# EternityJune25/ComoRAG

Hardware: NVIDIA H100
Metric: queries/sec (higher is better)
Workload: dtype bf16

## Files before the change

comorag_b200/csrc/common.cu:

```cuda
#include "common.cuh"

#include <stdarg.h>
#include <string.h>

#include <mutex>

namespace crag {

namespace {
thread_local char g_err[512] = {0};

typedef CUresult (*EncodeTiledFn)(CUtensorMap*, CUtensorMapDataType, cuuint32_t, void*, const cuuint64_t*,
                                  const cuuint64_t*, const cuuint32_t*, const cuuint32_t*, CUtensorMapInterleave,
                                  CUtensorMapSwizzle, CUtensorMapL2promotion, CUtensorMapFloatOOBfill);

EncodeTiledFn get_encode_fn() {
  static EncodeTiledFn fn = nullptr;
  static std::once_flag once;
  std::call_once(once, [] {
    void* p = nullptr;
    cudaDriverEntryPointQueryResult q;
    if (cudaGetDriverEntryPoint("cuTensorMapEncodeTiled", &p, cudaEnableDefault, &q) == cudaSuccess &&
        q == cudaDriverEntryPointSuccess)
      fn = reinterpret_cast<EncodeTiledFn>(p);
  });
  return fn;
}
}

void set_error(const char* fmt, ...) {
  va_list ap;
  va_start(ap, fmt);
  vsnprintf(g_err, sizeof(g_err), fmt, ap);
  va_end(ap);
}

int fail(int code, const char* fmt, ...) {
  va_list ap;
  va_start(ap, fmt);
  vsnprintf(g_err, sizeof(g_err), fmt, ap);
  va_end(ap);
  return code;
}

int make_tmap_bf16_2d(CUtensorMap* out, const void* base, uint64_t rows, uint64_t cols, uint64_t row_stride_bytes,
                      uint32_t box_rows, uint32_t box_cols) {
  EncodeTiledFn enc = get_encode_fn();
  if (!enc) return fail(CRAG_ERR_CUDA, "cuTensorMapEncodeTiled entry point unavailable (driver too old?)");
  if (rows == 0 || cols == 0) return fail(CRAG_ERR_INVALID, "tensor map over an empty tensor");
  const cuuint64_t gdim[2] = {cols, rows};
  const cuuint64_t gstride[1] = {row_stride_bytes};
  const cuuint32_t box[2] = {box_cols, box_rows};
  const cuuint32_t estride[2] = {1, 1};
  CUresult r = enc(out, CU_TENSOR_MAP_DATA_TYPE_BFLOAT16, 2, const_cast<void*>(base), gdim, gstride, box, estride,
                   CU_TENSOR_MAP_INTERLEAVE_NONE, CU_TENSOR_MAP_SWIZZLE_128B, CU_TENSOR_MAP_L2_PROMOTION_L2_256B,
                   CU_TENSOR_MAP_FLOAT_OOB_FILL_NONE);
  if (r != CUDA_SUCCESS)
    return fail(CRAG_ERR_CUDA, "cuTensorMapEncodeTiled failed (CUresult %d; rows=%llu cols=%llu stride=%llu box=%ux%u)",
                int(r), (unsigned long long)rows, (unsigned long long)cols, (unsigned long long)row_stride_bytes,
                box_rows, box_cols);
  return CRAG_OK;
}

int sm_count() {
  static int cached[64] = {0};
  int dev = 0;
  cudaError_t e = cudaGetDevice(&dev);
  if (e != cudaSuccess || dev < 0 || dev >= 64) {
    fail(CRAG_ERR_CUDA, "no usable CUDA device (%s)", e != cudaSuccess ? cudaGetErrorString(e) : "device ordinal out of range");
    return -1;
  }
  if (cached[dev] == 0) {
    int n = 0;
    e = cudaDeviceGetAttribute(&n, cudaDevAttrMultiProcessorCount, dev);
    if (e != cudaSuccess) {
      fail(CRAG_ERR_CUDA, "cudaDeviceGetAttribute: %s", cudaGetErrorString(e));
      return -1;
    }
    cached[dev] = n;
  }
  return cached[dev];
}

}

extern "C" int crag_version(void) { return 1002; }
extern "C" const char* crag_last_error(void) { return crag::g_err; }
extern "C" int crag_sm_count(void) { return crag::sm_count(); }

namespace crag {
namespace {
struct VmemApi {
  CUresult (*reserve)(CUdeviceptr*, size_t, size_t, CUdeviceptr, unsigned long long) = nullptr;
  CUresult (*addr_free)(CUdeviceptr, size_t) = nullptr;
  CUresult (*create)(CUmemGenericAllocationHandle*, size_t, const CUmemAllocationProp*, unsigned long long) = nullptr;
  CUresult (*release)(CUmemGenericAllocationHandle) = nullptr;
  CUresult (*map)(CUdeviceptr, size_t, size_t, CUmemGenericAllocationHandle, unsigned long long) = nullptr;
  CUresult (*unmap)(CUdeviceptr, size_t) = nullptr;
  CUresult (*set_access)(CUdeviceptr, size_t, const CUmemAccessDesc*, size_t) = nullptr;
  CUresult (*granularity)(size_t*, const CUmemAllocationProp*, CUmemAllocationGranularity_flags) = nullptr;
  bool ok = false;
};

const VmemApi& vmem_api() {
  static VmemApi api;
  static std::once_flag once;
  std::call_once(once, [] {
    auto get = [](const char* name, void** fn) {
      cudaDriverEntryPointQueryResult q;
      return cudaGetDriverEntryPoint(name, fn, cudaEnableDefault, &q) == cudaSuccess && q == cudaDriverEntryPointSuccess;
    };
    api.ok = get("cuMemAddressReserve", reinterpret_cast<void**>(&api.reserve)) &&
             get("cuMemAddressFree", reinterpret_cast<void**>(&api.addr_free)) &&
             get("cuMemCreate", reinterpret_cast<void**>(&api.create)) &&
             get("cuMemRelease", reinterpret_cast<void**>(&api.release)) &&
             get("cuMemMap", reinterpret_cast<void**>(&api.map)) &&
             get("cuMemUnmap", reinterpret_cast<void**>(&api.unmap)) &&
             get("cuMemSetAccess", reinterpret_cast<void**>(&api.set_access)) &&
             get("cuMemGetAllocationGranularity", reinterpret_cast<void**>(&api.granularity));
  });
  return api;
}

CUmemAllocationProp vmem_prop(int dev) {
  CUmemAllocationProp prop = {};
  prop.type = CU_MEM_ALLOCATION_TYPE_PINNED;
  prop.location.type = CU_MEM_LOCATION_TYPE_DEVICE;
  prop.location.id = dev;
  return prop;
}
}
}

extern "C" int crag_vmem_reserve(size_t max_bytes, uint64_t* base_out, size_t* granularity_out) {
  using namespace crag;
  const VmemApi& api = vmem_api();
  if (!api.ok) return fail(CRAG_ERR_UNSUPPORTED, "virtual memory management entry points unavailable");
  if (!base_out || !granularity_out || max_bytes == 0) return fail(CRAG_ERR_INVALID, "crag_vmem_reserve: bad arguments");
  int dev = 0;
  CRAG_CUDA_OK(cudaGetDevice(&dev));
  CRAG_CUDA_OK(cudaFree(nullptr));
  const CUmemAllocationProp prop = vmem_prop(dev);
  size_t gran = 0;
  CUresult r = api.granularity(&gran, &prop, CU_MEM_ALLOC_GRANULARITY_RECOMMENDED);
  if (r != CUDA_SUCCESS || gran == 0) return fail(CRAG_ERR_CUDA, "cuMemGetAllocationGranularity failed (%d)", int(r));
  const size_t size = (max_bytes + gran - 1) / gran * gran;
  CUdeviceptr base = 0;
  r = api.reserve(&base, size, gran, 0, 0);
  if (r != CUDA_SUCCESS) return fail(CRAG_ERR_CUDA, "cuMemAddressReserve(%zu) failed (%d)", size, int(r));
  *base_out = uint64_t(base);
  *granularity_out = gran;
  return CRAG_OK;
}

extern "C" int crag_vmem_grow(uint64_t base, size_t mapped_bytes, size_t new_mapped_bytes) {
  using namespace crag;
  const VmemApi& api = vmem_api();
  if (!api.ok) return fail(CRAG_ERR_UNSUPPORTED, "virtual memory management entry points unavailable");
  if (new_mapped_bytes <= mapped_bytes) return CRAG_OK;
  int dev = 0;
  CRAG_CUDA_OK(cudaGetDevice(&dev));
  const CUmemAllocationProp prop = vmem_prop(dev);
  const size_t bytes = new_mapped_bytes - mapped_bytes;
  CUmemGenericAllocationHandle h;
  CUresult r = api.create(&h, bytes, &prop, 0);
  if (r != CUDA_SUCCESS) return fail(CRAG_ERR_CUDA, "cuMemCreate(%zu) failed (%d): out of device memory?", bytes, int(r));
  r = api.map(CUdeviceptr(base + mapped_bytes), bytes, 0, h, 0);
  if (r != CUDA_SUCCESS) {
    api.release(h);
    return fail(CRAG_ERR_CUDA, "cuMemMap failed (%d)", int(r));
  }
  api.release(h);
  CUmemAccessDesc acc = {};
  acc.location.type = CU_MEM_LOCATION_TYPE_DEVICE;
  acc.location.id = dev;
  acc.flags = CU_MEM_ACCESS_FLAGS_PROT_READWRITE;
  r = api.set_access(CUdeviceptr(base + mapped_bytes), bytes, &acc, 1);
  if (r != CUDA_SUCCESS) return fail(CRAG_ERR_CUDA, "cuMemSetAccess failed (%d)", int(r));
  return CRAG_OK;
}

extern "C" int crag_vmem_release(uint64_t base, size_t mapped_bytes, size_t reserved_bytes) {
  using namespace crag;
  const VmemApi& api = vmem_api();
  if (!api.ok) return fail(CRAG_ERR_UNSUPPORTED, "virtual memory management entry points unavailable");
  if (mapped_bytes) {
    CUresult r = api.unmap(CUdeviceptr(base), mapped_bytes);
    if (r != CUDA_SUCCESS) return fail(CRAG_ERR_CUDA, "cuMemUnmap failed (%d)", int(r));
  }
  CUresult r = api.addr_free(CUdeviceptr(base), reserved_bytes);
  if (r != CUDA_SUCCESS) return fail(CRAG_ERR_CUDA, "cuMemAddressFree failed (%d)", int(r));
  return CRAG_OK;
}
```

comorag_b200/csrc/gemm.cu:

```cuda
#include <cstdlib>

#include "common.cuh"
#include "gemm.cuh"
#include "ptx.cuh"

namespace crag {

constexpr int kGemmBM = 128;
constexpr int kGemmBN = 128;
constexpr int kGemmBK = 64;
constexpr int kGemmConsumerWarps = 8;
constexpr int kGemmThreads = 32 * kGemmConsumerWarps + 32;
constexpr int kGemmStages = 3;

struct GemmLayout {
  static constexpr int kABytes = kGemmBM * kGemmBK * 2;
  static constexpr int kBBytes = kGemmBN * kGemmBK * 2;
  static constexpr int kStageBytes = kABytes + kBBytes;
  static constexpr size_t smem_bytes() { return 1024 + size_t(kGemmStages) * kStageBytes + 2 * kGemmStages * 8; }
};

__device__ __forceinline__ float gelu_erf(float x) {
  const float z = x * 0.70710678118654752f;
  const float az = fabsf(z);
  float t;
  asm("rcp.approx.ftz.f32 %0, %1;" : "=f"(t) : "f"(fmaf(0.3275911f, az, 1.0f)));
  float p = fmaf(1.061405429f, t, -1.453152027f);
  p = fmaf(p, t, 1.421413741f);
  p = fmaf(p, t, -0.284496736f);
  p = fmaf(p, t, 0.254829592f);
  p *= t;
  float e;
  asm("ex2.approx.ftz.f32 %0, %1;" : "=f"(e) : "f"(az * az * -1.4426950408889634f));
  const float erf_abs = fmaf(-p, e, 1.0f);
  const float half_x = 0.5f * x;
  return fmaf(half_x, copysignf(erf_abs, z), half_x);
}

__device__ __forceinline__ uint32_t pack_bf16x2(float a, float b) {
  __nv_bfloat162 v = __floats2bfloat162_rn(a, b);
  return *reinterpret_cast<uint32_t*>(&v);
}

template <int EPI>
__global__ void __launch_bounds__(kGemmThreads, 2)
gemm_bf16_kernel(const __grid_constant__ CUtensorMap tm_a, const __grid_constant__ CUtensorMap tm_b, int M, int N,
                 int K, const float* __restrict__ bias, const __nv_bfloat16* __restrict__ residual, int64_t ldr,
                 __nv_bfloat16* __restrict__ out, int64_t ldo) {
  using L = GemmLayout;
  constexpr int STAGES = kGemmStages;
  extern __shared__ uint8_t smem_raw[];
  uint8_t* smem = reinterpret_cast<uint8_t*>((reinterpret_cast<uintptr_t>(smem_raw) + 1023) & ~uintptr_t(1023));
  uint64_t* bar_full = reinterpret_cast<uint64_t*>(smem + STAGES * L::kStageBytes);
  uint64_t* bar_empty = bar_full + STAGES;

  const int warp = threadIdx.x >> 5;
  const int lane = threadIdx.x & 31;
  int n_blk = blockIdx.x, m_blk = blockIdx.y;
  if constexpr (EPI == GEMM_EPI_SCORES_F32) {
    const int m_blocks = (M + kGemmBM - 1) / kGemmBM;
    m_blk = int(blockIdx.x % unsigned(m_blocks));
    n_blk = int(blockIdx.x / unsigned(m_blocks));
  }
  const int num_kb = (K + kGemmBK - 1) / kGemmBK;

  if (threadIdx.x == 0) {
    for (int s = 0; s < STAGES; ++s) {
      mbar_init(&bar_full[s], 1);
      mbar_init(&bar_empty[s], kGemmConsumerWarps);
    }
    fence_mbar_init();
  }
  __syncthreads();

  if (warp == kGemmConsumerWarps) {
    if (lane == 0) {
      tma_prefetch_desc(&tm_a);
      tma_prefetch_desc(&tm_b);
      const uint64_t pol_w = policy_evict_last();
      int stage = 0;
      uint32_t phase = 0;
      for (int kb = 0; kb < num_kb; ++kb) {
        mbar_wait(&bar_empty[stage], phase ^ 1);
        uint8_t* sa = smem + stage * L::kStageBytes;
        mbar_arrive_expect_tx(&bar_full[stage], L::kStageBytes);
        tma_load_2d(&tm_a, &bar_full[stage], sa, kb * kGemmBK, m_blk * kGemmBM);
        tma_load_2d_hint(&tm_b, &bar_full[stage], sa + L::kABytes, kb * kGemmBK, n_blk * kGemmBN, pol_w);
        if (++stage == STAGES) { stage = 0; phase ^= 1; }
      }
    }
    return;
  }

  const int wg = warp >> 2;
  float acc[kGemmBN / 2];
#pragma unroll
  for (int i = 0; i < kGemmBN / 2; ++i) acc[i] = 0.f;
  int stage = 0, prev = 0;
  uint32_t phase = 0;
  for (int kb = 0; kb < num_kb; ++kb) {
    mbar_wait(&bar_full[stage], phase);
    const uint32_t a_addr = smem_u32(smem + stage * L::kStageBytes) + wg * 64 * 128;
    const uint32_t b_addr = smem_u32(smem + stage * L::kStageBytes + L::kABytes);
    wgmma_fence();
#pragma unroll
    for (int ks = 0; ks < kGemmBK / 16; ++ks)
      wgmma_m64n128k16_ss(acc, wgmma_desc_sw128(a_addr + ks * 32), wgmma_desc_sw128(b_addr + ks * 32), 1u);
    wgmma_commit();
    wgmma_wait<1>();
    if (kb > 0 && lane == 0) mbar_arrive(&bar_empty[prev]);
    prev = stage;
    if (++stage == STAGES) { stage = 0; phase ^= 1; }
  }
  wgmma_wait<0>();
  wgmma_fence_regs(acc);

  if constexpr (EPI == GEMM_EPI_SCORES_F32) {
    float* outf = reinterpret_cast<float*>(out);
    const int srow0 = m_blk * kGemmBM + wg * 64 + (warp & 3) * 16 + (lane >> 2);
    const int scol0 = n_blk * kGemmBN + 2 * (lane & 3);
#pragma unroll
    for (int j = 0; j < kGemmBN / 8; ++j) {
      const int col = scol0 + 8 * j;
#pragma unroll
      for (int h = 0; h < 2; ++h) {
        const int row = srow0 + 8 * h;
        if (row >= M) continue;
        float* p = outf + int64_t(row) * ldo + col;
        if (col + 1 < N) *reinterpret_cast<float2*>(p) = make_float2(acc[4 * j + 2 * h], acc[4 * j + 2 * h + 1]);
        else if (col < N) p[0] = acc[4 * j + 2 * h];
      }
    }
    return;
  }

  const int row0 = m_blk * kGemmBM + wg * 64 + (warp & 3) * 16 + (lane >> 2);
  const int col0 = n_blk * kGemmBN + 2 * (lane & 3);
#pragma unroll
  for (int j = 0; j < kGemmBN / 8; ++j) {
    const int col = col0 + 8 * j;
    if (col >= N) continue;
    const float2 b = __ldg(reinterpret_cast<const float2*>(bias + col));
#pragma unroll
    for (int h = 0; h < 2; ++h) {
      const int row = row0 + 8 * h;
      if (row >= M) continue;
      float x0 = acc[4 * j + 2 * h] + b.x, x1 = acc[4 * j + 2 * h + 1] + b.y;
      if (EPI == GEMM_EPI_BIAS_GELU) {
        x0 = gelu_erf(x0);
        x1 = gelu_erf(x1);
      }
      if (EPI == GEMM_EPI_BIAS_RESIDUAL) {
        const __nv_bfloat162 r = *reinterpret_cast<const __nv_bfloat162*>(residual + int64_t(row) * ldr + col);
        x0 += __bfloat162float(r.x);
        x1 += __bfloat162float(r.y);
      }
      *reinterpret_cast<uint32_t*>(out + int64_t(row) * ldo + col) = pack_bf16x2(x0, x1);
    }
  }
}

template <int EPI>
static int launch_gemm_t(const CUtensorMap& tm_a, const CUtensorMap& tm_b, int M, int N, int K, const float* bias,
                         const __nv_bfloat16* residual, int64_t ldr, __nv_bfloat16* out, int64_t ldo,
                         cudaStream_t stream) {
  auto kern = gemm_bf16_kernel<EPI>;
  {
    static bool done[64] = {false};
    int dev = 0;
    CRAG_CUDA_OK(cudaGetDevice(&dev));
    if (dev < 0 || dev >= 64 || !done[dev]) {
      CRAG_CUDA_OK(cudaFuncSetAttribute(kern, cudaFuncAttributeMaxDynamicSharedMemorySize, int(GemmLayout::smem_bytes())));
      if (dev >= 0 && dev < 64) done[dev] = true;
    }
  }
  const unsigned n_blocks = (N + kGemmBN - 1) / kGemmBN, m_blocks = (M + kGemmBM - 1) / kGemmBM;
  const dim3 grid = EPI == GEMM_EPI_SCORES_F32 ? dim3(m_blocks * n_blocks) : dim3(n_blocks, m_blocks);
  kern<<<grid, kGemmThreads, GemmLayout::smem_bytes(), stream>>>(tm_a, tm_b, M, N, K, bias, residual, ldr, out, ldo);
  CRAG_CUDA_OK(cudaGetLastError());
  return CRAG_OK;
}

int gemm_bf16(const void* a, int64_t lda, const void* w, int64_t ldw, const float* bias, const void* residual,
              int64_t ldr, void* out, int64_t ldo, int M, int N, int K, int epi, cudaStream_t stream) {
  if (M <= 0) return CRAG_OK;
  if (N < 8 || K < 8 || N % 8 != 0 || K % 8 != 0) return fail(CRAG_ERR_INVALID, "gemm: N and K must be positive multiples of 8 (N=%d K=%d)", N, K);
  if (lda % 8 || ldw % 8 || ldo % 8 || (epi == GEMM_EPI_BIAS_RESIDUAL && ldr % 8)) return fail(CRAG_ERR_INVALID, "gemm: leading dimensions must be multiples of 8 elements");
  if (!a || !w || !bias || !out || (epi == GEMM_EPI_BIAS_RESIDUAL && !residual)) return fail(CRAG_ERR_INVALID, "gemm: null pointer");
  if ((uintptr_t(a) | uintptr_t(w) | uintptr_t(out) | uintptr_t(bias) | uintptr_t(residual)) & 15) return fail(CRAG_ERR_INVALID, "gemm: pointers must be 16-byte aligned");
  if ((M + kGemmBM - 1) / kGemmBM > 65535) return fail(CRAG_ERR_INVALID, "gemm: M too large (%d)", M);
  const __nv_bfloat16* res = static_cast<const __nv_bfloat16*>(residual);
  __nv_bfloat16* o = static_cast<__nv_bfloat16*>(out);
  CUtensorMap tm_a, tm_b;
  int rc = make_tmap_bf16_2d(&tm_a, a, uint64_t(M), uint64_t(K), uint64_t(lda) * 2, kGemmBM);
  if (rc != CRAG_OK) return rc;
  rc = make_tmap_bf16_2d(&tm_b, w, uint64_t(N), uint64_t(K), uint64_t(ldw) * 2, kGemmBN);
  if (rc != CRAG_OK) return rc;
  switch (epi) {
    case GEMM_EPI_BIAS: return launch_gemm_t<GEMM_EPI_BIAS>(tm_a, tm_b, M, N, K, bias, res, ldr, o, ldo, stream);
    case GEMM_EPI_BIAS_GELU: return launch_gemm_t<GEMM_EPI_BIAS_GELU>(tm_a, tm_b, M, N, K, bias, res, ldr, o, ldo, stream);
    case GEMM_EPI_BIAS_RESIDUAL: return launch_gemm_t<GEMM_EPI_BIAS_RESIDUAL>(tm_a, tm_b, M, N, K, bias, res, ldr, o, ldo, stream);
  }
  return fail(CRAG_ERR_INVALID, "gemm: unknown epilogue %d", epi);
}

int gemm_scores_f32(const void* a, int64_t lda, const void* w, int64_t ldw, float* out, int64_t ldo, int M, int N,
                    int K, cudaStream_t stream) {
  if (M <= 0 || N <= 0) return CRAG_OK;
  if (K < 64 || K % 64 != 0 || lda % 8 || ldw % 8 || ldo % 2) return fail(CRAG_ERR_INVALID, "gemm scores: K must be a multiple of 64, lda/ldw multiples of 8 and ldo even");
  if ((uintptr_t(a) | uintptr_t(w)) & 15 || uintptr_t(out) & 7) return fail(CRAG_ERR_INVALID, "gemm scores: misaligned pointer");
  if (int64_t((M + kGemmBM - 1) / kGemmBM) * ((N + kGemmBN - 1) / kGemmBN) > int64_t(0x7FFFFFFF)) return fail(CRAG_ERR_INVALID, "gemm scores: too many tiles (M=%d N=%d)", M, N);
  CUtensorMap tm_a, tm_b;
  int rc = make_tmap_bf16_2d(&tm_a, a, uint64_t(M), uint64_t(K), uint64_t(lda) * 2, kGemmBM);
  if (rc != CRAG_OK) return rc;
  rc = make_tmap_bf16_2d(&tm_b, w, uint64_t(N), uint64_t(K), uint64_t(ldw) * 2, kGemmBN);
  if (rc != CRAG_OK) return rc;
  return launch_gemm_t<GEMM_EPI_SCORES_F32>(tm_a, tm_b, M, N, K, nullptr, nullptr, 0, reinterpret_cast<__nv_bfloat16*>(out),
                                            ldo, stream);
}

}

extern "C" int crag_gemm_bf16(const void* a, int64_t lda, const void* w, int64_t ldw, const float* bias,
                              const void* residual, int64_t ldr, void* out, int64_t ldo, int m, int n, int k,
                              int epilogue, crag_stream_t stream) {
  return crag::gemm_bf16(a, lda, w, ldw, bias, residual, ldr, out, ldo, m, n, k, epilogue,
                         static_cast<cudaStream_t>(stream));
}
```

comorag_b200/csrc/ptx.cuh:

```cuda
#pragma once
#include <cuda.h>
#include <cuda_runtime.h>
#include <cuda_bf16.h>
#include <stdint.h>

namespace crag {

__device__ __forceinline__ uint32_t smem_u32(const void* p) {
  return static_cast<uint32_t>(__cvta_generic_to_shared(p));
}

__device__ __forceinline__ bool elect_one() {
  uint32_t pred = 0;
  asm volatile(
      "{\n\t.reg .pred p;\n\t"
      "elect.sync _|p, 0xffffffff;\n\t"
      "selp.u32 %0, 1, 0, p;\n\t}"
      : "=r"(pred));
  return pred != 0;
}

__device__ __forceinline__ void mbar_init(uint64_t* bar, uint32_t count) {
  asm volatile("mbarrier.init.shared::cta.b64 [%0], %1;" ::"r"(smem_u32(bar)), "r"(count));
}
__device__ __forceinline__ void fence_mbar_init() {
  asm volatile("fence.mbarrier_init.release.cluster;" ::: "memory");
}
__device__ __forceinline__ void fence_proxy_async() {
  asm volatile("fence.proxy.async.shared::cta;" ::: "memory");
}
__device__ __forceinline__ void mbar_arrive_expect_tx(uint64_t* bar, uint32_t bytes) {
  asm volatile("mbarrier.arrive.expect_tx.shared::cta.b64 _, [%0], %1;" ::"r"(smem_u32(bar)), "r"(bytes)
               : "memory");
}
__device__ __forceinline__ void mbar_arrive(uint64_t* bar) {
  asm volatile("mbarrier.arrive.shared::cta.b64 _, [%0];" ::"r"(smem_u32(bar)) : "memory");
}
__device__ __forceinline__ bool mbar_try_wait(uint64_t* bar, uint32_t parity) {
  uint32_t ok;
  asm volatile(
      "{\n\t.reg .pred p;\n\t"
      "mbarrier.try_wait.parity.shared::cta.b64 p, [%1], %2;\n\t"
      "selp.u32 %0, 1, 0, p;\n\t}"
      : "=r"(ok)
      : "r"(smem_u32(bar)), "r"(parity)
      : "memory");
  return ok != 0;
}
#ifndef CRAG_MBAR_SPIN_LIMIT
#define CRAG_MBAR_SPIN_LIMIT (1ll << 33)
#endif
__device__ __forceinline__ void mbar_wait(uint64_t* bar, uint32_t parity) {
  if (mbar_try_wait(bar, parity)) return;
  const long long t0 = clock64();
  uint32_t spins = 0;
  while (!mbar_try_wait(bar, parity)) {
    if ((++spins & 0x3FF) == 0 && clock64() - t0 > CRAG_MBAR_SPIN_LIMIT) __trap();
  }
}

__device__ __forceinline__ void tma_prefetch_desc(const CUtensorMap* m) {
  asm volatile("prefetch.tensormap [%0];" ::"l"(reinterpret_cast<uint64_t>(m)) : "memory");
}
__device__ __forceinline__ void tma_load_2d(const CUtensorMap* m, uint64_t* bar, void* dst, int32_t c0,
                                            int32_t c1) {
  asm volatile(
      "cp.async.bulk.tensor.2d.shared::cluster.global.mbarrier::complete_tx::bytes"
      " [%0], [%1, {%3, %4}], [%2];" ::"r"(smem_u32(dst)),
      "l"(reinterpret_cast<uint64_t>(m)), "r"(smem_u32(bar)), "r"(c0), "r"(c1)
      : "memory");
}
__device__ __forceinline__ void tma_load_2d_hint(const CUtensorMap* m, uint64_t* bar, void* dst, int32_t c0,
                                                 int32_t c1, uint64_t policy) {
  asm volatile(
      "cp.async.bulk.tensor.2d.shared::cluster.global.mbarrier::complete_tx::bytes.L2::cache_hint"
      " [%0], [%1, {%3, %4}], [%2], %5;" ::"r"(smem_u32(dst)),
      "l"(reinterpret_cast<uint64_t>(m)), "r"(smem_u32(bar)), "r"(c0), "r"(c1), "l"(policy)
      : "memory");
}
__device__ __forceinline__ uint64_t policy_evict_first() {
  uint64_t p;
  asm volatile("createpolicy.fractional.L2::evict_first.b64 %0, 1.0;" : "=l"(p));
  return p;
}
__device__ __forceinline__ uint64_t policy_evict_normal() {
  uint64_t p;
  asm volatile("createpolicy.fractional.L2::evict_normal.b64 %0, 1.0;" : "=l"(p));
  return p;
}
__device__ __forceinline__ uint64_t policy_evict_last() {
  uint64_t p;
  asm volatile("createpolicy.fractional.L2::evict_last.b64 %0, 1.0;" : "=l"(p));
  return p;
}

__device__ __forceinline__ void wgmma_fence() { asm volatile("wgmma.fence.sync.aligned;" ::: "memory"); }
__device__ __forceinline__ void wgmma_commit() { asm volatile("wgmma.commit_group.sync.aligned;" ::: "memory"); }
template <int N>
__device__ __forceinline__ void wgmma_wait() { asm volatile("wgmma.wait_group.sync.aligned %0;" ::"n"(N) : "memory"); }
template <int R>
__device__ __forceinline__ void wgmma_fence_regs(float (&d)[R]) {
#pragma unroll
  for (int i = 0; i < R; ++i) asm volatile("" : "+f"(d[i])::"memory");
}

__device__ __forceinline__ uint64_t wgmma_desc_sw128(uint32_t smem_addr) {
  uint64_t d = 0;
  d |= static_cast<uint64_t>((smem_addr & 0x3FFFF) >> 4);
  d |= static_cast<uint64_t>(1) << 16;
  d |= static_cast<uint64_t>(1024 >> 4) << 32;
  d |= static_cast<uint64_t>(1) << 62;
  return d;
}

__device__ __forceinline__ void wgmma_m64n32k16_ss(float (&d)[16], uint64_t desc_a, uint64_t desc_b, uint32_t accumulate) {
  asm volatile(
      "{\n\t.reg .pred p;\n\t"
      "setp.ne.b32 p, %18, 0;\n\t"
      "wgmma.mma_async.sync.aligned.m64n32k16.f32.bf16.bf16 "
      "{%0, %1, %2, %3, %4, %5, %6, %7, %8, %9, %10, %11, %12, %13, %14, %15}, %16, %17, p, 1, 1, 0, 0;\n\t}"
      : "+f"(d[0]), "+f"(d[1]), "+f"(d[2]), "+f"(d[3]), "+f"(d[4]), "+f"(d[5]), "+f"(d[6]), "+f"(d[7]), "+f"(d[8]), "+f"(d[9]), "+f"(d[10]), "+f"(d[11]), "+f"(d[12]), "+f"(d[13]), "+f"(d[14]), "+f"(d[15])
      : "l"(desc_a), "l"(desc_b), "r"(accumulate));
}
__device__ __forceinline__ void wgmma_m64n64k16_ss(float (&d)[32], uint64_t desc_a, uint64_t desc_b, uint32_t accumulate) {
  asm volatile(
      "{\n\t.reg .pred p;\n\t"
      "setp.ne.b32 p, %34, 0;\n\t"
      "wgmma.mma_async.sync.aligned.m64n64k16.f32.bf16.bf16 "
      "{%0, %1, %2, %3, %4, %5, %6, %7, %8, %9, %10, %11, %12, %13, %14, %15, %16, %17, %18, %19, %20, %21, %22, %23, %24, %25, %26, %27, %28, %29, %30, %31}, %32, %33, p, 1, 1, 0, 0;\n\t}"
      : "+f"(d[0]), "+f"(d[1]), "+f"(d[2]), "+f"(d[3]), "+f"(d[4]), "+f"(d[5]), "+f"(d[6]), "+f"(d[7]), "+f"(d[8]), "+f"(d[9]), "+f"(d[10]), "+f"(d[11]), "+f"(d[12]), "+f"(d[13]), "+f"(d[14]), "+f"(d[15]), "+f"(d[16]), "+f"(d[17]), "+f"(d[18]), "+f"(d[19]), "+f"(d[20]), "+f"(d[21]), "+f"(d[22]), "+f"(d[23]), "+f"(d[24]), "+f"(d[25]), "+f"(d[26]), "+f"(d[27]), "+f"(d[28]), "+f"(d[29]), "+f"(d[30]), "+f"(d[31])
      : "l"(desc_a), "l"(desc_b), "r"(accumulate));
}
__device__ __forceinline__ void wgmma_m64n128k16_ss(float (&d)[64], uint64_t desc_a, uint64_t desc_b, uint32_t accumulate) {
  asm volatile(
      "{\n\t.reg .pred p;\n\t"
      "setp.ne.b32 p, %66, 0;\n\t"
      "wgmma.mma_async.sync.aligned.m64n128k16.f32.bf16.bf16 "
      "{%0, %1, %2, %3, %4, %5, %6, %7, %8, %9, %10, %11, %12, %13, %14, %15, %16, %17, %18, %19, %20, %21, %22, %23, %24, %25, %26, %27, %28, %29, %30, %31, %32, %33, %34, %35, %36, %37, %38, %39, %40, %41, %42, %43, %44, %45, %46, %47, %48, %49, %50, %51, %52, %53, %54, %55, %56, %57, %58, %59, %60, %61, %62, %63}, %64, %65, p, 1, 1, 0, 0;\n\t}"
      : "+f"(d[0]), "+f"(d[1]), "+f"(d[2]), "+f"(d[3]), "+f"(d[4]), "+f"(d[5]), "+f"(d[6]), "+f"(d[7]), "+f"(d[8]), "+f"(d[9]), "+f"(d[10]), "+f"(d[11]), "+f"(d[12]), "+f"(d[13]), "+f"(d[14]), "+f"(d[15]), "+f"(d[16]), "+f"(d[17]), "+f"(d[18]), "+f"(d[19]), "+f"(d[20]), "+f"(d[21]), "+f"(d[22]), "+f"(d[23]), "+f"(d[24]), "+f"(d[25]), "+f"(d[26]), "+f"(d[27]), "+f"(d[28]), "+f"(d[29]), "+f"(d[30]), "+f"(d[31]), "+f"(d[32]), "+f"(d[33]), "+f"(d[34]), "+f"(d[35]), "+f"(d[36]), "+f"(d[37]), "+f"(d[38]), "+f"(d[39]), "+f"(d[40]), "+f"(d[41]), "+f"(d[42]), "+f"(d[43]), "+f"(d[44]), "+f"(d[45]), "+f"(d[46]), "+f"(d[47]), "+f"(d[48]), "+f"(d[49]), "+f"(d[50]), "+f"(d[51]), "+f"(d[52]), "+f"(d[53]), "+f"(d[54]), "+f"(d[55]), "+f"(d[56]), "+f"(d[57]), "+f"(d[58]), "+f"(d[59]), "+f"(d[60]), "+f"(d[61]), "+f"(d[62]), "+f"(d[63])
      : "l"(desc_a), "l"(desc_b), "r"(accumulate));
}
__device__ __forceinline__ void wgmma_m64n64k16_rs_bmn(float (&d)[32], const uint32_t (&a)[4], uint64_t desc_b,
                                                      uint32_t accumulate) {
  asm volatile(
      "{\n\t.reg .pred p;\n\t"
      "setp.ne.b32 p, %37, 0;\n\t"
      "wgmma.mma_async.sync.aligned.m64n64k16.f32.bf16.bf16 "
      "{%0, %1, %2, %3, %4, %5, %6, %7, %8, %9, %10, %11, %12, %13, %14, %15, %16, %17, %18, %19, %20, %21, %22, %23, %24, %25, %26, %27, %28, %29, %30, %31}, {%32, %33, %34, %35}, %36, p, 1, 1, 1;\n\t}"
      : "+f"(d[0]), "+f"(d[1]), "+f"(d[2]), "+f"(d[3]), "+f"(d[4]), "+f"(d[5]), "+f"(d[6]), "+f"(d[7]), "+f"(d[8]), "+f"(d[9]), "+f"(d[10]), "+f"(d[11]), "+f"(d[12]), "+f"(d[13]), "+f"(d[14]), "+f"(d[15]), "+f"(d[16]), "+f"(d[17]), "+f"(d[18]), "+f"(d[19]), "+f"(d[20]), "+f"(d[21]), "+f"(d[22]), "+f"(d[23]), "+f"(d[24]), "+f"(d[25]), "+f"(d[26]), "+f"(d[27]), "+f"(d[28]), "+f"(d[29]), "+f"(d[30]), "+f"(d[31])
      : "r"(a[0]), "r"(a[1]), "r"(a[2]), "r"(a[3]), "l"(desc_b), "r"(accumulate));
}

}
```

Before: 4462.

## Make GEMM persistent with warp-specialized epilogue, deeper pipeline, and adaptive BN

Turns the GEMM into a persistent kernel with one grid-sized loop over output tiles. Separate producer, consumer and epilogue warp roles hand off through mbarriers and a swizzled fp32 shared-memory staging buffer, so the epilogue of one tile can overlap the main loop of the next. It also halves BK to 32 using 64B swizzle, raises the stage count to fill shared memory, rebalances registers with setmaxnreg, and picks BN=256 or 128 based on the tile count. The risks are lower occupancy (one CTA per SM), extra shared-memory traffic for staging, and a serialization point on the single staging buffer.

Result: no change. 4457, median of 6 (-0.1%).

```diff
diff --git a/comorag_b200/csrc/common.cu b/comorag_b200/csrc/common.cu
--- a/comorag_b200/csrc/common.cu
+++ b/comorag_b200/csrc/common.cu
@@ -53,7 +53,7 @@
   const cuuint32_t box[2] = {box_cols, box_rows};
   const cuuint32_t estride[2] = {1, 1};
   CUresult r = enc(out, CU_TENSOR_MAP_DATA_TYPE_BFLOAT16, 2, const_cast<void*>(base), gdim, gstride, box, estride,
-                   CU_TENSOR_MAP_INTERLEAVE_NONE, CU_TENSOR_MAP_SWIZZLE_128B, CU_TENSOR_MAP_L2_PROMOTION_L2_256B,
+                   CU_TENSOR_MAP_INTERLEAVE_NONE, box_cols == 32 ? CU_TENSOR_MAP_SWIZZLE_64B : CU_TENSOR_MAP_SWIZZLE_128B, CU_TENSOR_MAP_L2_PROMOTION_L2_256B,
                    CU_TENSOR_MAP_FLOAT_OOB_FILL_NONE);
   if (r != CUDA_SUCCESS)
     return fail(CRAG_ERR_CUDA, "cuTensorMapEncodeTiled failed (CUresult %d; rows=%llu cols=%llu stride=%llu box=%ux%u)",
diff --git a/comorag_b200/csrc/gemm.cu b/comorag_b200/csrc/gemm.cu
--- a/comorag_b200/csrc/gemm.cu
+++ b/comorag_b200/csrc/gemm.cu
@@ -1,23 +1,31 @@
+#include <algorithm>
 #include <cstdlib>
 
 #include "common.cuh"
 #include "gemm.cuh"
+#include "gemm_pipeline.cuh"
 #include "ptx.cuh"
 
 namespace crag {
 
 constexpr int kGemmBM = 128;
-constexpr int kGemmBN = 128;
-constexpr int kGemmBK = 64;
+constexpr int kGemmBK = 32;
 constexpr int kGemmConsumerWarps = 8;
-constexpr int kGemmThreads = 32 * kGemmConsumerWarps + 32;
-constexpr int kGemmStages = 3;
-
+constexpr int kGemmEpilogueWarps = 3;
+constexpr int kGemmEpilogueRows = 4;
+constexpr int kGemmThreads = 32 * (1 + kGemmEpilogueWarps + kGemmConsumerWarps);
+constexpr int kGemmSmemLimit = 232448;
+
+template <int BN>
 struct GemmLayout {
   static constexpr int kABytes = kGemmBM * kGemmBK * 2;
-  static constexpr int kBBytes = kGemmBN * kGemmBK * 2;
+  static constexpr int kBBytes = BN * kGemmBK * 2;
   static constexpr int kStageBytes = kABytes + kBBytes;
-  static constexpr size_t smem_bytes() { return 1024 + size_t(kGemmStages) * kStageBytes + 2 * kGemmStages * 8; }
+  static constexpr int kStagingBytes = kGemmBM * BN * 4;
+  static constexpr int kBarBytes = 256;
+  static constexpr int kStages = std::min(8, (kGemmSmemLimit - 1024 - kStagingBytes - kBarBytes) / kStageBytes);
+  static constexpr size_t smem_bytes() { return 1024 + size_t(kStages) * kStageBytes + kStagingBytes + kBarBytes; }
+  static_assert(kStages >= 3 && smem_bytes() <= size_t(kGemmSmemLimit), "GEMM shared memory");
 };
 
 __device__ __forceinline__ float gelu_erf(float x) {
@@ -42,143 +50,232 @@
   return *reinterpret_cast<uint32_t*>(&v);
 }
 
-template <int EPI>
-__global__ void __launch_bounds__(kGemmThreads, 2)
+template <int BN>
+__device__ __forceinline__ float* staging_chunk(float* staging, int r, int chunk) {
+  return staging + r * BN + ((chunk ^ (r & 7)) << 3);
+}
+
+struct GemmBars {
+  uint64_t* full;
+  uint64_t* empty;
+  uint64_t* staged;
+  uint64_t* drained;
+  int lane;
+  __device__ __forceinline__ void wait_empty(int s, uint32_t parity) { mbar_wait(&empty[s], parity); }
+  __device__ __forceinline__ void wait_full(int s, uint32_t parity) { mbar_wait(&full[s], parity); }
+  __device__ __forceinline__ void release(int s) { if (lane == 0) mbar_arrive(&empty[s]); }
+  __device__ __forceinline__ void wait_staging_empty(uint32_t parity) { mbar_wait(drained, parity); }
+  __device__ __forceinline__ void staging_full() { mbar_arrive(staged); }
+  __device__ __forceinline__ void wait_staging_full(uint32_t parity) { mbar_wait(staged, parity); }
+  __device__ __forceinline__ void staging_empty() { mbar_arrive(drained); }
+};
+
+template <int BN, int EPI>
+__device__ __forceinline__ void gemm_epilogue_tile(float* staging, int ew, int lane, int m_blk, int n_blk, int M,
+                                                   int N, const float* __restrict__ bias,
+                                                   const __nv_bfloat16* __restrict__ residual, int64_t ldr,
+                                                   __nv_bfloat16* __restrict__ out, int64_t ldo) {
+  constexpr int kThreadsPerRow = BN / 8;
+  constexpr int kRowsPerPass = 32 / kThreadsPerRow;
+  const int chunk = lane % kThreadsPerRow;
+  const int col = n_blk * BN + 8 * chunk;
+  const int r_first = ew * kRowsPerPass + lane / kThreadsPerRow;
+  constexpr int kRowStep = kGemmEpilogueWarps * kRowsPerPass;
+  if constexpr (EPI == GEMM_EPI_SCORES_F32) {
+    float* outf = reinterpret_cast<float*>(out);
+    for (int r = r_first; r < kGemmBM; r += kRowStep) {
+      const int row = m_blk * kGemmBM + r;
+      if (row >= M) break;
+      const float* src = staging_chunk<BN>(staging, r, chunk);
+      float v[8];
+      *reinterpret_cast<float4*>(v) = *reinterpret_cast<const float4*>(src);
+      *reinterpret_cast<float4*>(v + 4) = *reinterpret_cast<const float4*>(src + 4);
+      float* p = outf + int64_t(row) * ldo + col;
+#pragma unroll
+      for (int e = 0; e < 8; e += 2) {
+        if (col + e + 1 < N) *reinterpret_cast<float2*>(p + e) = make_float2(v[e], v[e + 1]);
+        else if (col + e < N) p[e] = v[e];
+      }
+    }
+    return;
+  }
+  if (col >= N) return;
+  float b[8];
+  *reinterpret_cast<float4*>(b) = __ldg(reinterpret_cast<const float4*>(bias + col));
+  *reinterpret_cast<float4*>(b + 4) = __ldg(reinterpret_cast<const float4*>(bias + col + 4));
+  constexpr int U = kGemmEpilogueRows;
+  for (int r = r_first; r < kGemmBM; r += U * kRowStep) {
+    float x[U][8];
+    uint4 res_v[U];
+    bool live[U];
+#pragma unroll
+    for (int u = 0; u < U; ++u) {
+      const int rr = r + u * kRowStep;
+      const int row = m_blk * kGemmBM + rr;
+      live[u] = rr < kGemmBM && row < M;
+      if (!live[u]) continue;
+      const float* src = staging_chunk<BN>(staging, rr, chunk);
+      *reinterpret_cast<float4*>(x[u]) = *reinterpret_cast<const float4*>(src);
+      *reinterpret_cast<float4*>(x[u] + 4) = *reinterpret_cast<const float4*>(src + 4);
+      if constexpr (EPI == GEMM_EPI_BIAS_RESIDUAL)
+        res_v[u] = *reinterpret_cast<const uint4*>(residual + int64_t(row) * ldr + col);
+    }
+    if (!live[0]) break;
+#pragma unroll
+    for (int u = 0; u < U; ++u) {
+      if (!live[u]) continue;
+      const __nv_bfloat16* res_h = reinterpret_cast<const __nv_bfloat16*>(&res_v[u]);
+      uint32_t packed[4];
+#pragma unroll
+      for (int e = 0; e < 8; e += 2) {
+        float x0 = x[u][e] + b[e], x1 = x[u][e + 1] + b[e + 1];
+        if constexpr (EPI == GEMM_EPI_BIAS_GELU) {
+          x0 = gelu_erf(x0);
+          x1 = gelu_erf(x1);
+        }
+        if constexpr (EPI == GEMM_EPI_BIAS_RESIDUAL) {
+          x0 += __bfloat162float(res_h[e]);
+          x1 += __bfloat162float(res_h[e + 1]);
+        }
+        packed[e / 2] = pack_bf16x2(x0, x1);
+      }
+      const int row = m_blk * kGemmBM + r + u * kRowStep;
+      *reinterpret_cast<uint4*>(out + int64_t(row) * ldo + col) = make_uint4(packed[0], packed[1], packed[2], packed[3]);
+    }
+  }
+}
+
+template <int BN>
+__device__ __forceinline__ void wgmma_tile(float (&acc)[BN / 2], uint64_t desc_a, uint64_t desc_b) {
+  if constexpr (BN == 256) wgmma_m64n256k16_ss(acc, desc_a, desc_b, 1u);
+  else wgmma_m64n128k16_ss(acc, desc_a, desc_b, 1u);
+}
+
+template <int BN, int EPI>
+__global__ void __launch_bounds__(kGemmThreads, 1)
 gemm_bf16_kernel(const __grid_constant__ CUtensorMap tm_a, const __grid_constant__ CUtensorMap tm_b, int M, int N,
                  int K, const float* __restrict__ bias, const __nv_bfloat16* __restrict__ residual, int64_t ldr,
                  __nv_bfloat16* __restrict__ out, int64_t ldo) {
-  using L = GemmLayout;
-  constexpr int STAGES = kGemmStages;
+  using L = GemmLayout<BN>;
+  constexpr int S = L::kStages;
   extern __shared__ uint8_t smem_raw[];
   uint8_t* smem = reinterpret_cast<uint8_t*>((reinterpret_cast<uintptr_t>(smem_raw) + 1023) & ~uintptr_t(1023));
-  uint64_t* bar_full = reinterpret_cast<uint64_t*>(smem + STAGES * L::kStageBytes);
-  uint64_t* bar_empty = bar_full + STAGES;
+  float* staging = reinterpret_cast<float*>(smem + S * L::kStageBytes);
+  uint64_t* bar_full = reinterpret_cast<uint64_t*>(smem + S * L::kStageBytes + L::kStagingBytes);
+  uint64_t* bar_empty = bar_full + S;
 
   const int warp = threadIdx.x >> 5;
   const int lane = threadIdx.x & 31;
-  int n_blk = blockIdx.x, m_blk = blockIdx.y;
-  if constexpr (EPI == GEMM_EPI_SCORES_F32) {
-    const int m_blocks = (M + kGemmBM - 1) / kGemmBM;
-    m_blk = int(blockIdx.x % unsigned(m_blocks));
-    n_blk = int(blockIdx.x / unsigned(m_blocks));
-  }
-  const int num_kb = (K + kGemmBK - 1) / kGemmBK;
+  const GemmTileSchedule sched{(M + kGemmBM - 1) / kGemmBM, (N + BN - 1) / BN, (K + kGemmBK - 1) / kGemmBK,
+                               EPI == GEMM_EPI_SCORES_F32};
+  GemmBars bars{bar_full, bar_empty, bar_empty + S, bar_empty + S + 1, lane};
 
   if (threadIdx.x == 0) {
-    for (int s = 0; s < STAGES; ++s) {
+    for (int s = 0; s < S; ++s) {
       mbar_init(&bar_full[s], 1);
       mbar_init(&bar_empty[s], kGemmConsumerWarps);
     }
+    mbar_init(bars.staged, 32 * kGemmConsumerWarps);
+    mbar_init(bars.drained, 32 * kGemmEpilogueWarps);
     fence_mbar_init();
   }
   __syncthreads();
 
-  if (warp == kGemmConsumerWarps) {
-    if (lane == 0) {
-      tma_prefetch_desc(&tm_a);
-      tma_prefetch_desc(&tm_b);
-      const uint64_t pol_w = policy_evict_last();
-      int stage = 0;
-      uint32_t phase = 0;
-      for (int kb = 0; kb < num_kb; ++kb) {
-        mbar_wait(&bar_empty[stage], phase ^ 1);
-        uint8_t* sa = smem + stage * L::kStageBytes;
-        mbar_arrive_expect_tx(&bar_full[stage], L::kStageBytes);
-        tma_load_2d(&tm_a, &bar_full[stage], sa, kb * kGemmBK, m_blk * kGemmBM);
-        tma_load_2d_hint(&tm_b, &bar_full[stage], sa + L::kABytes, kb * kGemmBK, n_blk * kGemmBN, pol_w);
-        if (++stage == STAGES) { stage = 0; phase ^= 1; }
+  if (warp < 4) {
+    setmaxnreg_dec<96>();
+    if (warp == 0) {
+      if (lane == 0) {
+        tma_prefetch_desc(&tm_a);
+        tma_prefetch_desc(&tm_b);
+        const uint64_t pol_w = policy_evict_last();
+        gemm_producer_role<S>(sched, blockIdx.x, gridDim.x, bars, [&](int st, int m_blk, int n_blk, int kb) {
+          uint8_t* sa = smem + st * L::kStageBytes;
+          mbar_arrive_expect_tx(&bar_full[st], L::kStageBytes);
+          tma_load_2d(&tm_a, &bar_full[st], sa, kb * kGemmBK, m_blk * kGemmBM);
+          tma_load_2d_hint(&tm_b, &bar_full[st], sa + L::kABytes, kb * kGemmBK, n_blk * BN, pol_w);
+        });
       }
-    }
+      return;
+    }
+    gemm_epilogue_role(sched, blockIdx.x, gridDim.x, bars, [&](int m_blk, int n_blk) {
+      gemm_epilogue_tile<BN, EPI>(staging, warp - 1, lane, m_blk, n_blk, M, N, bias, residual, ldr, out, ldo);
+    });
     return;
   }
 
-  const int wg = warp >> 2;
-  float acc[kGemmBN / 2];
-#pragma unroll
-  for (int i = 0; i < kGemmBN / 2; ++i) acc[i] = 0.f;
-  int stage = 0, prev = 0;
-  uint32_t phase = 0;
-  for (int kb = 0; kb < num_kb; ++kb) {
-    mbar_wait(&bar_full[stage], phase);
-    const uint32_t a_addr = smem_u32(smem + stage * L::kStageBytes) + wg * 64 * 128;
-    const uint32_t b_addr = smem_u32(smem + stage * L::kStageBytes + L::kABytes);
-    wgmma_fence();
-#pragma unroll
-    for (int ks = 0; ks < kGemmBK / 16; ++ks)
-      wgmma_m64n128k16_ss(acc, wgmma_desc_sw128(a_addr + ks * 32), wgmma_desc_sw128(b_addr + ks * 32), 1u);
-    wgmma_commit();
-    wgmma_wait<1>();
-    if (kb > 0 && lane == 0) mbar_arrive(&bar_empty[prev]);
-    prev = stage;
-    if (++stage == STAGES) { stage = 0; phase ^= 1; }
-  }
-  wgmma_wait<0>();
-  wgmma_fence_regs(acc);
-
-  if constexpr (EPI == GEMM_EPI_SCORES_F32) {
-    float* outf = reinterpret_cast<float*>(out);
-    const int srow0 = m_blk * kGemmBM + wg * 64 + (warp & 3) * 16 + (lane >> 2);
-    const int scol0 = n_blk * kGemmBN + 2 * (lane & 3);
-#pragma unroll
-    for (int j = 0; j < kGemmBN / 8; ++j) {
-      const int col = scol0 + 8 * j;
-#pragma unroll
-      for (int h = 0; h < 2; ++h) {
-        const int row = srow0 + 8 * h;
-        if (row >= M) continue;
-        float* p = outf + int64_t(row) * ldo + col;
-        if (col + 1 < N) *reinterpret_cast<float2*>(p) = make_float2(acc[4 * j + 2 * h], acc[4 * j + 2 * h + 1]);
-        else if (col < N) p[0] = acc[4 * j + 2 * h];
-      }
-    }
-    return;
-  }
-
-  const int row0 = m_blk * kGemmBM + wg * 64 + (warp & 3) * 16 + (lane >> 2);
-  const int col0 = n_blk * kGemmBN + 2 * (lane & 3);
-#pragma unroll
-  for (int j = 0; j < kGemmBN / 8; ++j) {
-    const int col = col0 + 8 * j;
-    if (col >= N) continue;
-    const float2 b = __ldg(reinterpret_cast<const float2*>(bias + col));
-#pragma unroll
-    for (int h = 0; h < 2; ++h) {
-      const int row = row0 + 8 * h;
-      if (row >= M) continue;
-      float x0 = acc[4 * j + 2 * h] + b.x, x1 = acc[4 * j + 2 * h + 1] + b.y;
-      if (EPI == GEMM_EPI_BIAS_GELU) {
-        x0 = gelu_erf(x0);
-        x1 = gelu_erf(x1);
-      }
-      if (EPI == GEMM_EPI_BIAS_RESIDUAL) {
-        const __nv_bfloat162 r = *reinterpret_cast<const __nv_bfloat162*>(residual + int64_t(row) * ldr + col);
-        x0 += __bfloat162float(r.x);
-        x1 += __bfloat162float(r.y);
-      }
-      *reinterpret_cast<uint32_t*>(out + int64_t(row) * ldo + col) = pack_bf16x2(x0, x1);
-    }
-  }
-}
-
-template <int EPI>
-static int launch_gemm_t(const CUtensorMap& tm_a, const CUtensorMap& tm_b, int M, int N, int K, const float* bias,
-                         const __nv_bfloat16* residual, int64_t ldr, __nv_bfloat16* out, int64_t ldo,
-                         cudaStream_t stream) {
-  auto kern = gemm_bf16_kernel<EPI>;
+  setmaxnreg_inc<200>();
+  const int wg = (warp >> 2) - 1;
+  float acc[BN / 2];
+  gemm_consumer_role<S>(
+      sched, blockIdx.x, gridDim.x, bars,
+      [&] {
+#pragma unroll
+        for (int i = 0; i < BN / 2; ++i) acc[i] = 0.f;
+      },
+      [&](int st, int) {
+        const uint32_t a_addr = smem_u32(smem + st * L::kStageBytes) + wg * 64 * (kGemmBK * 2);
+        const uint32_t b_addr = smem_u32(smem + st * L::kStageBytes + L::kABytes);
+        wgmma_fence();
+#pragma unroll
+        for (int ks = 0; ks < kGemmBK / 16; ++ks)
+          wgmma_tile<BN>(acc, wgmma_desc_sw64(a_addr + ks * 32), wgmma_desc_sw64(b_addr + ks * 32));
+        wgmma_commit();
+        wgmma_wait<1>();
+      },
+      [&] {
+        wgmma_wait<0>();
+        wgmma_fence_regs(acc);
+      },
+      [&](int, int) {
+        const int r0 = wg * 64 + (warp & 3) * 16 + (lane >> 2);
+#pragma unroll
+        for (int j = 0; j < BN / 8; ++j) {
+#pragma unroll
+          for (int h = 0; h < 2; ++h) {
+            float* p = staging_chunk<BN>(staging, r0 + 8 * h, j) + 2 * (lane & 3);
+            *reinterpret_cast<float2*>(p) = make_float2(acc[4 * j + 2 * h], acc[4 * j + 2 * h + 1]);
+          }
+        }
+      });
+}
+
+template <int BN, int EPI>
+static int launch_gemm_bn(const void* a, int64_t lda, const void* w, int64_t ldw, int M, int N, int K,
+                          const float* bias, const __nv_bfloat16* residual, int64_t ldr, __nv_bfloat16* out,
+                          int64_t ldo, int sms, cudaStream_t stream) {
+  using L = GemmLayout<BN>;
+  auto kern = gemm_bf16_kernel<BN, EPI>;
   {
     static bool done[64] = {false};
     int dev = 0;
     CRAG_CUDA_OK(cudaGetDevice(&dev));
     if (dev < 0 || dev >= 64 || !done[dev]) {
-      CRAG_CUDA_OK(cudaFuncSetAttribute(kern, cudaFuncAttributeMaxDynamicSharedMemorySize, int(GemmLayout::smem_bytes())));
+      CRAG_CUDA_OK(cudaFuncSetAttribute(kern, cudaFuncAttributeMaxDynamicSharedMemorySize, int(L::smem_bytes())));
       if (dev >= 0 && dev < 64) done[dev] = true;
     }
   }
-  const unsigned n_blocks = (N + kGemmBN - 1) / kGemmBN, m_blocks = (M + kGemmBM - 1) / kGemmBM;
-  const dim3 grid = EPI == GEMM_EPI_SCORES_F32 ? dim3(m_blocks * n_blocks) : dim3(n_blocks, m_blocks);
-  kern<<<grid, kGemmThreads, GemmLayout::smem_bytes(), stream>>>(tm_a, tm_b, M, N, K, bias, residual, ldr, out, ldo);
+  CUtensorMap tm_a, tm_b;
+  int rc = make_tmap_bf16_2d(&tm_a, a, uint64_t(M), uint64_t(K), uint64_t(lda) * 2, kGemmBM, kGemmBK);
+  if (rc != CRAG_OK) return rc;
+  rc = make_tmap_bf16_2d(&tm_b, w, uint64_t(N), uint64_t(K), uint64_t(ldw) * 2, BN, kGemmBK);
+  if (rc != CRAG_OK) return rc;
+  const int64_t tiles = int64_t((M + kGemmBM - 1) / kGemmBM) * ((N + BN - 1) / BN);
+  const unsigned grid = unsigned(std::min<int64_t>(tiles, sms));
+  kern<<<grid, kGemmThreads, L::smem_bytes(), stream>>>(tm_a, tm_b, M, N, K, bias, residual, ldr, out, ldo);
   CRAG_CUDA_OK(cudaGetLastError());
   return CRAG_OK;
+}
+
+template <int EPI>
+static int launch_gemm(const void* a, int64_t lda, const void* w, int64_t ldw, int M, int N, int K, const float* bias,
+                       const __nv_bfloat16* residual, int64_t ldr, __nv_bfloat16* out, int64_t ldo,
+                       cudaStream_t stream) {
+  const int sms = sm_count();
+  if (sms <= 0) return CRAG_ERR_CUDA;
+  const int64_t tiles256 = int64_t((M + kGemmBM - 1) / kGemmBM) * ((N + 255) / 256);
+  if (tiles256 >= sms)
+    return launch_gemm_bn<256, EPI>(a, lda, w, ldw, M, N, K, bias, residual, ldr, out, ldo, sms, stream);
+  return launch_gemm_bn<128, EPI>(a, lda, w, ldw, M, N, K, bias, residual, ldr, out, ldo, sms, stream);
 }
 
 int gemm_bf16(const void* a, int64_t lda, const void* w, int64_t ldw, const float* bias, const void* residual,
@@ -191,15 +288,10 @@
   if ((M + kGemmBM - 1) / kGemmBM > 65535) return fail(CRAG_ERR_INVALID, "gemm: M too large (%d)", M);
   const __nv_bfloat16* res = static_cast<const __nv_bfloat16*>(residual);
   __nv_bfloat16* o = static_cast<__nv_bfloat16*>(out);
-  CUtensorMap tm_a, tm_b;
-  int rc = make_tmap_bf16_2d(&tm_a, a, uint64_t(M), uint64_t(K), uint64_t(lda) * 2, kGemmBM);
-  if (rc != CRAG_OK) return rc;
-  rc = make_tmap_bf16_2d(&tm_b, w, uint64_t(N), uint64_t(K), uint64_t(ldw) * 2, kGemmBN);
-  if (rc != CRAG_OK) return rc;
   switch (epi) {
-    case GEMM_EPI_BIAS: return launch_gemm_t<GEMM_EPI_BIAS>(tm_a, tm_b, M, N, K, bias, res, ldr, o, ldo, stream);
-    case GEMM_EPI_BIAS_GELU: return launch_gemm_t<GEMM_EPI_BIAS_GELU>(tm_a, tm_b, M, N, K, bias, res, ldr, o, ldo, stream);
-    case GEMM_EPI_BIAS_RESIDUAL: return launch_gemm_t<GEMM_EPI_BIAS_RESIDUAL>(tm_a, tm_b, M, N, K, bias, res, ldr, o, ldo, stream);
+    case GEMM_EPI_BIAS: return launch_gemm<GEMM_EPI_BIAS>(a, lda, w, ldw, M, N, K, bias, res, ldr, o, ldo, stream);
+    case GEMM_EPI_BIAS_GELU: return launch_gemm<GEMM_EPI_BIAS_GELU>(a, lda, w, ldw, M, N, K, bias, res, ldr, o, ldo, stream);
+    case GEMM_EPI_BIAS_RESIDUAL: return launch_gemm<GEMM_EPI_BIAS_RESIDUAL>(a, lda, w, ldw, M, N, K, bias, res, ldr, o, ldo, stream);
   }
   return fail(CRAG_ERR_INVALID, "gemm: unknown epilogue %d", epi);
 }
@@ -209,14 +301,9 @@
   if (M <= 0 || N <= 0) return CRAG_OK;
   if (K < 64 || K % 64 != 0 || lda % 8 || ldw % 8 || ldo % 2) return fail(CRAG_ERR_INVALID, "gemm scores: K must be a multiple of 64, lda/ldw multiples of 8 and ldo even");
   if ((uintptr_t(a) | uintptr_t(w)) & 15 || uintptr_t(out) & 7) return fail(CRAG_ERR_INVALID, "gemm scores: misaligned pointer");
-  if (int64_t((M + kGemmBM - 1) / kGemmBM) * ((N + kGemmBN - 1) / kGemmBN) > int64_t(0x7FFFFFFF)) return fail(CRAG_ERR_INVALID, "gemm scores: too many tiles (M=%d N=%d)", M, N);
-  CUtensorMap tm_a, tm_b;
-  int rc = make_tmap_bf16_2d(&tm_a, a, uint64_t(M), uint64_t(K), uint64_t(lda) * 2, kGemmBM);
-  if (rc != CRAG_OK) return rc;
-  rc = make_tmap_bf16_2d(&tm_b, w, uint64_t(N), uint64_t(K), uint64_t(ldw) * 2, kGemmBN);
-  if (rc != CRAG_OK) return rc;
-  return launch_gemm_t<GEMM_EPI_SCORES_F32>(tm_a, tm_b, M, N, K, nullptr, nullptr, 0, reinterpret_cast<__nv_bfloat16*>(out),
-                                            ldo, stream);
+  if (int64_t((M + kGemmBM - 1) / kGemmBM) * ((N + 127) / 128) > int64_t(0x7FFFFFFF)) return fail(CRAG_ERR_INVALID, "gemm scores: too many tiles (M=%d N=%d)", M, N);
+  return launch_gemm<GEMM_EPI_SCORES_F32>(a, lda, w, ldw, M, N, K, nullptr, nullptr, 0, reinterpret_cast<__nv_bfloat16*>(out),
+                                         ldo, stream);
 }
 
 }
diff --git a/comorag_b200/csrc/gemm_pipeline.cuh b/comorag_b200/csrc/gemm_pipeline.cuh
--- /dev/null
+++ b/comorag_b200/csrc/gemm_pipeline.cuh
@@ -0,0 +1,94 @@
+#pragma once
+#include <stdint.h>
+
+#ifdef __CUDACC__
+#define CRAG_PIPE_FN __host__ __device__ __forceinline__
+#else
+#define CRAG_PIPE_FN inline
+#endif
+
+namespace crag {
+
+struct GemmTileSchedule {
+  int m_blocks, n_blocks, num_kb;
+  bool m_fastest;
+
+  CRAG_PIPE_FN int64_t tiles() const { return int64_t(m_blocks) * n_blocks; }
+  CRAG_PIPE_FN void coords(int64_t t, int& m, int& n) const {
+    if (m_fastest) {
+      m = int(t % m_blocks);
+      n = int(t / m_blocks);
+    } else {
+      n = int(t % n_blocks);
+      m = int(t / n_blocks);
+    }
+  }
+};
+
+template <int S>
+struct RingPos {
+  int stage = 0;
+  uint32_t phase = 0;
+  CRAG_PIPE_FN void advance() {
+    if (++stage == S) {
+      stage = 0;
+      phase ^= 1;
+    }
+  }
+};
+
+template <int S, class Bars, class Load>
+CRAG_PIPE_FN void gemm_producer_role(const GemmTileSchedule& s, int64_t cta, int64_t grid, Bars& bars, Load&& load) {
+  RingPos<S> p;
+  for (int64_t t = cta; t < s.tiles(); t += grid) {
+    int m, n;
+    s.coords(t, m, n);
+    for (int kb = 0; kb < s.num_kb; ++kb) {
+      bars.wait_empty(p.stage, p.phase ^ 1);
+      load(p.stage, m, n, kb);
+      p.advance();
+    }
+  }
+}
+
+template <int S, class Bars, class Begin, class Mma, class Drain, class ToStaging>
+CRAG_PIPE_FN void gemm_consumer_role(const GemmTileSchedule& s, int64_t cta, int64_t grid, Bars& bars, Begin&& begin,
+                                     Mma&& mma, Drain&& drain, ToStaging&& to_staging) {
+  RingPos<S> p;
+  uint32_t staging_phase = 0;
+  for (int64_t t = cta; t < s.tiles(); t += grid) {
+    int m, n;
+    s.coords(t, m, n);
+    begin();
+    int prev = 0;
+    for (int kb = 0; kb < s.num_kb; ++kb) {
+      bars.wait_full(p.stage, p.phase);
+      mma(p.stage, kb);
+      if (kb > 0) bars.release(prev);
+      prev = p.stage;
+      p.advance();
+    }
+    drain();
+    bars.release(prev);
+    bars.wait_staging_empty(staging_phase ^ 1);
+    to_staging(m, n);
+    bars.staging_full();
+    staging_phase ^= 1;
+  }
+}
+
+template <class Bars, class Epilogue>
+CRAG_PIPE_FN void gemm_epilogue_role(const GemmTileSchedule& s, int64_t cta, int64_t grid, Bars& bars,
+                                     Epilogue&& epilogue) {
+  uint32_t staging_phase = 0;
+  for (int64_t t = cta; t < s.tiles(); t += grid) {
+    int m, n;
+    s.coords(t, m, n);
+    bars.wait_staging_full(staging_phase);
+    epilogue(m, n);
+    bars.staging_empty();
+    staging_phase ^= 1;
+  }
+}
+
+}
diff --git a/comorag_b200/csrc/ptx.cuh b/comorag_b200/csrc/ptx.cuh
--- a/comorag_b200/csrc/ptx.cuh
+++ b/comorag_b200/csrc/ptx.cuh
@@ -113,6 +113,20 @@
   return d;
 }
 
+__device__ __forceinline__ uint64_t wgmma_desc_sw64(uint32_t smem_addr) {
+  uint64_t d = 0;
+  d |= static_cast<uint64_t>((smem_addr & 0x3FFFF) >> 4);
+  d |= static_cast<uint64_t>(1) << 16;
+  d |= static_cast<uint64_t>(512 >> 4) << 32;
+  d |= static_cast<uint64_t>(2) << 62;
+  return d;
+}
+
+template <int N>
+__device__ __forceinline__ void setmaxnreg_dec() { asm volatile("setmaxnreg.dec.sync.aligned.u32 %0;" ::"n"(N)); }
+template <int N>
+__device__ __forceinline__ void setmaxnreg_inc() { asm volatile("setmaxnreg.inc.sync.aligned.u32 %0;" ::"n"(N)); }
+
 __device__ __forceinline__ void wgmma_m64n32k16_ss(float (&d)[16], uint64_t desc_a, uint64_t desc_b, uint32_t accumulate) {
   asm volatile(
       "{\n\t.reg .pred p;\n\t"
@@ -140,6 +154,15 @@
       : "+f"(d[0]), "+f"(d[1]), "+f"(d[2]), "+f"(d[3]), "+f"(d[4]), "+f"(d[5]), "+f"(d[6]), "+f"(d[7]), "+f"(d[8]), "+f"(d[9]), "+f"(d[10]), "+f"(d[11]), "+f"(d[12]), "+f"(d[13]), "+f"(d[14]), "+f"(d[15]), "+f"(d[16]), "+f"(d[17]), "+f"(d[18]), "+f"(d[19]), "+f"(d[20]), "+f"(d[21]), "+f"(d[22]), "+f"(d[23]), "+f"(d[24]), "+f"(d[25]), "+f"(d[26]), "+f"(d[27]), "+f"(d[28]), "+f"(d[29]), "+f"(d[30]), "+f"(d[31]), "+f"(d[32]), "+f"(d[33]), "+f"(d[34]), "+f"(d[35]), "+f"(d[36]), "+f"(d[37]), "+f"(d[38]), "+f"(d[39]), "+f"(d[40]), "+f"(d[41]), "+f"(d[42]), "+f"(d[43]), "+f"(d[44]), "+f"(d[45]), "+f"(d[46]), "+f"(d[47]), "+f"(d[48]), "+f"(d[49]), "+f"(d[50]), "+f"(d[51]), "+f"(d[52]), "+f"(d[53]), "+f"(d[54]), "+f"(d[55]), "+f"(d[56]), "+f"(d[57]), "+f"(d[58]), "+f"(d[59]), "+f"(d[60]), "+f"(d[61]), "+f"(d[62]), "+f"(d[63])
       : "l"(desc_a), "l"(desc_b), "r"(accumulate));
 }
+__device__ __forceinline__ void wgmma_m64n256k16_ss(float (&d)[128], uint64_t desc_a, uint64_t desc_b, uint32_t accumulate) {
+  asm volatile(
+      "{\n\t.reg .pred p;\n\t"
+      "setp.ne.b32 p, %130, 0;\n\t"
+      "wgmma.mma_async.sync.aligned.m64n256k16.f32.bf16.bf16 "
+      "{%0, %1, %2, %3, %4, %5, %6, %7, %8, %9, %10, %11, %12, %13, %14, %15, %16, %17, %18, %19, %20, %21, %22, %23, %24, %25, %26, %27, %28, %29, %30, %31, %32, %33, %34, %35, %36, %37, %38, %39, %40, %41, %42, %43, %44, %45, %46, %47, %48, %49, %50, %51, %52, %53, %54, %55, %56, %57, %58, %59, %60, %61, %62, %63, %64, %65, %66, %67, %68, %69, %70, %71, %72, %73, %74, %75, %76, %77, %78, %79, %80, %81, %82, %83, %84, %85, %86, %87, %88, %89, %90, %91, %92, %93, %94, %95, %96, %97, %98, %99, %100, %101, %102, %103, %104, %105, %106, %107, %108, %109, %110, %111, %112, %113, %114, %115, %116, %117, %118, %119, %120, %121, %122, %123, %124, %125, %126, %127}, %128, %129, p, 1, 1, 0, 0;\n\t}"
+      : "+f"(d[0]), "+f"(d[1]), "+f"(d[2]), "+f"(d[3]), "+f"(d[4]), "+f"(d[5]), "+f"(d[6]), "+f"(d[7]), "+f"(d[8]), "+f"(d[9]), "+f"(d[10]), "+f"(d[11]), "+f"(d[12]), "+f"(d[13]), "+f"(d[14]), "+f"(d[15]), "+f"(d[16]), "+f"(d[17]), "+f"(d[18]), "+f"(d[19]), "+f"(d[20]), "+f"(d[21]), "+f"(d[22]), "+f"(d[23]), "+f"(d[24]), "+f"(d[25]), "+f"(d[26]), "+f"(d[27]), "+f"(d[28]), "+f"(d[29]), "+f"(d[30]), "+f"(d[31]), "+f"(d[32]), "+f"(d[33]), "+f"(d[34]), "+f"(d[35]), "+f"(d[36]), "+f"(d[37]), "+f"(d[38]), "+f"(d[39]), "+f"(d[40]), "+f"(d[41]), "+f"(d[42]), "+f"(d[43]), "+f"(d[44]), "+f"(d[45]), "+f"(d[46]), "+f"(d[47]), "+f"(d[48]), "+f"(d[49]), "+f"(d[50]), "+f"(d[51]), "+f"(d[52]), "+f"(d[53]), "+f"(d[54]), "+f"(d[55]), "+f"(d[56]), "+f"(d[57]), "+f"(d[58]), "+f"(d[59]), "+f"(d[60]), "+f"(d[61]), "+f"(d[62]), "+f"(d[63]), "+f"(d[64]), "+f"(d[65]), "+f"(d[66]), "+f"(d[67]), "+f"(d[68]), "+f"(d[69]), "+f"(d[70]), "+f"(d[71]), "+f"(d[72]), "+f"(d[73]), "+f"(d[74]), "+f"(d[75]), "+f"(d[76]), "+f"(d[77]), "+f"(d[78]), "+f"(d[79]), "+f"(d[80]), "+f"(d[81]), "+f"(d[82]), "+f"(d[83]), "+f"(d[84]), "+f"(d[85]), "+f"(d[86]), "+f"(d[87]), "+f"(d[88]), "+f"(d[89]), "+f"(d[90]), "+f"(d[91]), "+f"(d[92]), "+f"(d[93]), "+f"(d[94]), "+f"(d[95]), "+f"(d[96]), "+f"(d[97]), "+f"(d[98]), "+f"(d[99]), "+f"(d[100]), "+f"(d[101]), "+f"(d[102]), "+f"(d[103]), "+f"(d[104]), "+f"(d[105]), "+f"(d[106]), "+f"(d[107]), "+f"(d[108]), "+f"(d[109]), "+f"(d[110]), "+f"(d[111]), "+f"(d[112]), "+f"(d[113]), "+f"(d[114]), "+f"(d[115]), "+f"(d[116]), "+f"(d[117]), "+f"(d[118]), "+f"(d[119]), "+f"(d[120]), "+f"(d[121]), "+f"(d[122]), "+f"(d[123]), "+f"(d[124]), "+f"(d[125]), "+f"(d[126]), "+f"(d[127])
+      : "l"(desc_a), "l"(desc_b), "r"(accumulate));
+}
 __device__ __forceinline__ void wgmma_m64n64k16_rs_bmn(float (&d)[32], const uint32_t (&a)[4], uint64_t desc_b,
                                                       uint32_t accumulate) {
   asm volatile(
```
